# jiaozihao18/LC-Rec

Hardware: AMD Instinct MI355X
Metric: item-embeddings/sec through 4-level RQ encode+assign (higher is better)
Workload: dtype f32; 1 GPU; C3 synthetic 1M x 768-d, 4x256 codes; items_per_gpu=1000000, in_dim=768, e_dim=32, levels=4, codes_per_level=256, chunk_pipelines=1, bytes_per_item=3104

## Files before the change

### lc-rec_amd/csrc/gemm_f32.hip

```cpp
#include "common.h"

#include <stdlib.h>

namespace lcrec {

#ifdef LCREC_GEMM_STAMP
__device__ unsigned long long g_stamps[8][64][4];
__device__ unsigned long long g_marks[8][4];
#define LCREC_MARK(slot)                                                                           \
    do {                                                                                           \
        if (blockIdx.x == 8 && lane == 0) {                                                        \
            unsigned long long t_;                                                                 \
            asm volatile("s_memtime %0\n\ts_waitcnt lgkmcnt(0)" : "=s"(t_)::"memory");           \
            g_marks[wave][slot] = t_;                                                              \
        }                                                                                          \
    } while (0)
#define LCREC_STAMP(slot)                                                                          \
    do {                                                                                           \
        if (blockIdx.x == 8 && lane == 0 && 2 * u + half < 64) {                                   \
            unsigned long long t_;                                                                 \
            asm volatile("s_memtime %0\n\ts_waitcnt lgkmcnt(0)" : "=s"(t_)::"memory");           \
            g_stamps[wave][2 * u + half][slot] = t_;                                               \
        }                                                                                          \
    } while (0)
// ... 759 lines not shown
            for (int r = 0; r < 16; ++r) acc[i][j][r] = 0.f;

    const int nk = K / BKT;
    float *my_a = As0 + grp * GM * LDT;

    const __amdgpu_buffer_rsrc_t a_rsrc = tile_rsrc(A, m0, M, GM, K);
    const __amdgpu_buffer_rsrc_t w_rsrc = tile_rsrc(W, w_row0, N, 64, K);
    const int t_g = ((gt / KG) * K + (gt % KG) * 8) * 4;
    const int pass_g = RPI * K * 4;
    const uint32_t t_s = (uint32_t)(((gt / KG) * LDT + (gt % KG) * 8) * 4);
    uint32_t a_s[ITA], w_s[2][ITW];
#pragma unroll
    for (int it = 0; it < ITA; ++it) a_s[it] = lds_addr(my_a) + t_s + it * RPI * LDT * 4;
#pragma unroll
    for (int b = 0; b < 2; ++b)
#pragma unroll
        for (int it = 0; it < ITW; ++it) w_s[b][it] = lds_addr(Ws0 + b * BN * LDT + grp * 64 * LDT) + t_s + it * RPI * LDT * 4;

    f32x4 ra[ITA][2], rw[ITW][2];
    auto load_a = [&](int kt) {
#pragma unroll
        for (int it = 0; it < ITA; ++it) {
            const int so = kt * (BKT * 4) + it * pass_g;
            ra[it][0] = buffer_load_f32x4(a_rsrc, t_g, so);
            ra[it][1] = buffer_load_f32x4(a_rsrc, t_g + 16, so);
        }
    };
    auto load_w = [&](int kt) {
#pragma unroll
        for (int it = 0; it < ITW; ++it) {
            const int so = kt * (BKT * 4) + it * pass_g;
            rw[it][0] = buffer_load_f32x4(w_rsrc, t_g, so);
            rw[it][1] = buffer_load_f32x4(w_rsrc, t_g + 16, so);
        }
    };
    auto store_a = [&]() {
#pragma unroll
        for (int it = 0; it < ITA; ++it) lds_store_deint8(a_s[it], ra[it][0], ra[it][1]);
    };
    auto store_w = [&](int buf) {
#pragma unroll
        for (int it = 0; it < ITW; ++it) lds_store_deint8(w_s[buf][it], rw[it][0], rw[it][1]);
    };
    auto lds_drain = [&]() { asm volatile("s_waitcnt lgkmcnt(0)" ::: "memory"); };

    load_w(0);
    store_w(0);
    load_a(0);
    if (grp == 0) {
        store_a();
    } else if (nk > 1) {
        load_w(1);
    }
    lds_drain();
    __syncthreads();
    LCREC_MARK(1);

    const float *a_base = my_a + (wm * 64 + (lane & 31)) * LDT + (lane >> 5) * 4;
    const int w_off = (wn * 64 + (lane & 31)) * LDT + (lane >> 5) * 4;

    auto mfma_group = [&](const f32x4 (&af)[2], const f32x4 (&wf)[2]) {
#pragma unroll
        for (int q = 0; q < 4; ++q)
#pragma unroll
            for (int i = 0; i < 2; ++i)
#pragma unroll
                for (int j = 0; j < 2; ++j)
                    acc[i][j] = __builtin_amdgcn_mfma_f32_32x32x2f32(af[i][q], wf[j][q], acc[i][j], 0, 0, 0);
    };

    auto phase = [&](auto par_c, auto half_c, int u) {
        constexpr int PAR = decltype(par_c)::value, half = decltype(half_c)::value;
        if (grp == half) {
            LCREC_STAMP(0);
            const float *w_base = Ws0 + PAR * BN * LDT + w_off;
            f32x4 af[2][2], wf[2][2];
            auto frags = [&](int buf, int g) {
#pragma unroll
                for (int i = 0; i < 2; ++i) {
                    af[buf][i] = *reinterpret_cast<const f32x4 *>(a_base + i * 32 * LDT + g * 8);
                    wf[buf][i] = *reinterpret_cast<const f32x4 *>(w_base + i * 32 * LDT + g * 8);
                }
            };
            auto reads_then_mfmas = [&]() {
                __builtin_amdgcn_sched_group_barrier(0x100, 4, 0);
                __builtin_amdgcn_sched_group_barrier(0x008, 16, 0);
            };
            frags(0, 0);
            frags(1, 1);
            if (half == 0) {
                if (u + 1 < nk) { load_a(u + 1); load_w(u + 1); }
            } else {
                if (u + 1 < nk) load_a(u + 1);
                if (u + 2 < nk) load_w(u + 2);
            }
            __builtin_amdgcn_sched_barrier(0);
            mfma_group(af[0], wf[0]);
            __builtin_amdgcn_sched_barrier(0);
            frags(0, 2);
            mfma_group(af[1], wf[1]);
            reads_then_mfmas();
            __builtin_amdgcn_sched_barrier(0);
            frags(1, 3);
            mfma_group(af[0], wf[0]);
            reads_then_mfmas();
            __builtin_amdgcn_sched_barrier(0);
            LCREC_STAMP(1);
            __syncthreads();
            LCREC_STAMP(2);
            __builtin_amdgcn_s_setprio(3);
            mfma_group(af[1], wf[1]);
            __builtin_amdgcn_s_setprio(0);
            LCREC_STAMP(3);
        } else {
            LCREC_STAMP(0);
            store_a();
            store_w(PAR ^ 1);
            lds_drain();
            LCREC_STAMP(1);
            __syncthreads();
            LCREC_STAMP(2);
        }
    };

    for (int u = 0; u < nk; u += 2) {
        phase(IntC<0>{}, IntC<0>{}, u);
        phase(IntC<0>{}, IntC<1>{}, u);
        if (u + 1 < nk) {
            phase(IntC<1>{}, IntC<0>{}, u + 1);
            phase(IntC<1>{}, IntC<1>{}, u + 1);
        }
    }

    LCREC_MARK(2);
    float *stg = my_a + w4 * 32 * LDK;
#pragma unroll
    for (int j = 0; j < 2; ++j)
#pragma unroll
        for (int i = 0; i < 2; ++i)
            store_tile_32x32(acc[i][j], stg, lane, C, m0 + wm * 64 + i * 32, M, n0 + wn * 64 + j * 32, N, bias, bn_scale,
                             bn_shift, relu);
    LCREC_MARK(3);
}

typedef unsigned u32x4_t __attribute__((ext_vector_type(4)));

template <bool HAS_BN>
__global__ __launch_bounds__(512) void linear_fwd_pp3_kernel(
    const float *__restrict__ A, const float *__restrict__ W, const float *__restrict__ bias,
    const float *__restrict__ bn_scale, const float *__restrict__ bn_shift, float *__restrict__ C,
    int64_t M, int N, int K, int relu, int bn_blocks, int bm_blocks, int total_virtual, int xcd_order)
{
    constexpr int GM = 128, BN = 128, LDT = LDK;
    constexpr int STEADY = 0, HEAD0 = 1, HEAD_S0 = 2, HEAD_S8 = 10, TAIL0 = 11, TAIL1 = 12;
    extern __shared__ __attribute__((aligned(16))) float pp3_lds[];
    float *As0 = pp3_lds;
    float *Ws0 = As0 + 2 * GM * LDT;
    float *Ep0 = Ws0 + 2 * BN * LDT;

    const int tid = threadIdx.x, lane = tid & 63;
    const int wave = __builtin_amdgcn_readfirstlane(tid >> 6);
    const int grp = wave >> 2, w4 = wave & 3, wm = w4 >> 1, wn = w4 & 1;
    const int gt = tid & 255;
    const int nk = K / BK;
    float *my_a = As0 + grp * GM * LDT;
    float *patch = Ep0 + wave * 32 * LDT;

    auto tile_of = [&](int t, int64_t &o_m0, int &o_n0, int &o_arows, int &o_wrows) __attribute__((always_inline)) -> bool {
        int64_t bm;
        int bn;
        if (xcd_order) {
            const int xcd = t & 7, j = t >> 3;
            const int panels = (bm_blocks - xcd + 7) >> 3;
            if (j >= panels * bn_blocks) return false;
            bm = (int64_t)(j / bn_blocks) * 8 + xcd;
            bn = j % bn_blocks;
        } else {
            if (t >= bm_blocks * bn_blocks) return false;
            bm = t / bn_blocks;
            bn = t % bn_blocks;
        }
        o_m0 = bm * (2 * GM) + grp * GM;
        o_n0 = bn * BN;
        const int64_t ar = M - o_m0, wr = (int64_t)N - (o_n0 + grp * 64);
        o_arows = __builtin_amdgcn_readfirstlane((int)(ar < 0 ? 0 : (ar > GM ? GM : ar)));
        o_wrows = __builtin_amdgcn_readfirstlane((int)(wr < 0 ? 0 : (wr > 64 ? 64 : wr)));
        return true;
    };
    auto next_tile = [&](int t, int64_t &o_m0, int &o_n0, int &o_arows, int &o_wrows) __attribute__((always_inline)) -> int {
        for (t += gridDim.x; t < total_virtual; t += gridDim.x)
            if (tile_of(t, o_m0, o_n0, o_arows, o_wrows)) return t;
        return total_virtual;
    };

    int64_t cur_m0 = 0, nxt_m0 = 0, prv_m0 = 0;
    int cur_n0 = 0, nxt_n0 = 0, prv_n0 = 0, cur_ar = 0, nxt_ar = 0, prv_ar = 0, cur_wr = 0, nxt_wr = 0;
    int t = blockIdx.x;
    if (!tile_of(t, cur_m0, cur_n0, cur_ar, cur_wr)) t = next_tile(t, cur_m0, cur_n0, cur_ar, cur_wr);
    if (t >= total_virtual) return;
    int has_next = 0, have_prev = 0;

    const int t_g = ((gt >> 2) * K + (gt & 3) * 8) * 4;
    const int pass_g = 64 * K * 4;
    const uint32_t t_s = (uint32_t)(((gt >> 2) * LDT + (gt & 3) * 8) * 4);
    const uint32_t a_s0 = lds_addr(my_a) + t_s, a_s1 = a_s0 + 64 * LDT * 4;
    const uint32_t w_s[2] = {lds_addr(Ws0 + grp * 64 * LDT) + t_s, lds_addr(Ws0 + BN * LDT + grp * 64 * LDT) + t_s};

    __amdgpu_buffer_rsrc_t cur_a = tile_rsrc(A, cur_m0, M, GM, K), cur_w = tile_rsrc(W, cur_n0 + grp * 64, N, 64, K);
    __amdgpu_buffer_rsrc_t nxt_a = cur_a, nxt_w = cur_w;

    f32x4 ra[2][2], rw[2];
    auto load_a = [&](__amdgpu_buffer_rsrc_t r, int kt) __attribute__((always_inline)) {
        const int so = kt * (BK * 4);
        ra[0][0] = buffer_load_f32x4(r, t_g, so);
        ra[0][1] = buffer_load_f32x4(r, t_g + 16, so);
        ra[1][0] = buffer_load_f32x4(r, t_g, so + pass_g);
        ra[1][1] = buffer_load_f32x4(r, t_g + 16, so + pass_g);
    };
    auto load_w = [&](__amdgpu_buffer_rsrc_t r, int kt) __attribute__((always_inline)) {
        const int so = kt * (BK * 4);
        rw[0] = buffer_load_f32x4(r, t_g, so);
        rw[1] = buffer_load_f32x4(r, t_g + 16, so);
    };
    auto store_a = [&]() __attribute__((always_inline)) {
        lds_store_deint8(a_s0, ra[0][0], ra[0][1]);
        lds_store_deint8(a_s1, ra[1][0], ra[1][1]);
    };
    auto store_w = [&](int buf) __attribute__((always_inline)) { lds_store_deint8(w_s[buf], rw[0], rw[1]); };
    auto lds_drain = [&]() __attribute__((always_inline)) { asm volatile("s_waitcnt lgkmcnt(0)" ::: "memory"); };
    auto lds_barrier = [&]() __attribute__((always_inline)) { asm volatile("s_waitcnt lgkmcnt(0)\n\ts_barrier" ::: "memory"); };

    struct EpiConst { float b[2], sc[2], sh[2]; };
    auto load_epi = [&](EpiConst &e, int n0) __attribute__((always_inline)) {
#pragma unroll
        for (int j = 0; j < 2; ++j) {
            const int col = n0 + wn * 64 + j * 32 + (lane & 31);
            e.b[j] = bias ? bias[col] : 0.f;
            e.sc[j] = HAS_BN ? bn_scale[col] : 1.f;
            e.sh[j] = HAS_BN ? bn_shift[col] : 0.f;
        }
    };
    auto epi_math = [&](f32x16 (&dst)[2][2], const f32x16 (&src)[2][2], const EpiConst &e) __attribute__((always_inline)) {
#pragma unroll
        for (int i = 0; i < 2; ++i)
#pragma unroll
            for (int j = 0; j < 2; ++j)
#pragma unroll
                for (int r = 0; r < 16; ++r) {
                    float v = src[i][j][r] + e.b[j];
                    if (HAS_BN) v = __builtin_fmaf(v, e.sc[j], e.sh[j]);
                    if (relu) v = (v > 0.f) ? v : 0.f;
                    dst[i][j][r] = v;
                }
    };
    uint32_t patch_w = lds_addr(patch) + (uint32_t)((4 * (lane >> 5) * LDT + (lane & 31)) * 4);
    uint32_t patch_r = lds_addr(patch) + (uint32_t)(((lane >> 3) * LDT + (lane & 7) * 4) * 4);
    int c_voff = ((lane >> 3) * N + (lane & 7) * 4) * 4;
    asm volatile("" : "+v"(patch_w), "+v"(patch_r), "+v"(c_voff));
    auto epi_patch = [&](const f32x16 &v, auto hf_c) __attribute__((always_inline)) {
        constexpr int hf = decltype(hf_c)::value;
        const uint32_t pw = patch_w;
#define LCREC_PATCH_W(R)                                                                                         \
        asm volatile("ds_write_b32 %0, %1 offset:%2" ::"v"(pw), "v"(v[8 * hf + (R)]),                            \
                     "n"((((R) & 3) + 8 * ((8 * hf + (R)) >> 2)) * LDT * 4) : "memory")
        LCREC_PATCH_W(0); LCREC_PATCH_W(1); LCREC_PATCH_W(2); LCREC_PATCH_W(3);
        LCREC_PATCH_W(4); LCREC_PATCH_W(5); LCREC_PATCH_W(6); LCREC_PATCH_W(7);
#undef LCREC_PATCH_W
    };
    auto epi_send = [&](auto i_c, auto j_c, auto hf_c, int64_t t_m0, int t_n0, int rows) __attribute__((always_inline)) {
        constexpr int i = decltype(i_c)::value, j = decltype(j_c)::value, hf = decltype(hf_c)::value;
        const int extent = rows > 0 ? ((rows - 1) * N + BN) * 4 : 0;
        const __amdgpu_buffer_rsrc_t c_rsrc =
            __builtin_amdgcn_make_buffer_rsrc(C + t_m0 * (int64_t)N + t_n0, 0, extent, 0x00020000);
        f32x4 q[2];
        asm volatile("s_waitcnt lgkmcnt(0)\n\t"
                     "ds_read_b128 %0, %2 offset:%3\n\t"
                     "ds_read_b128 %1, %2 offset:%4\n\t"
                     "s_waitcnt lgkmcnt(0)"
                     : "=&v"(q[0]), "=&v"(q[1])
                     : "v"(patch_r), "n"((2 * hf) * 8 * LDT * 4), "n"((2 * hf + 1) * 8 * LDT * 4)
                     : "memory");
#pragma unroll
        for (int p = 0; p < 2; ++p) {
            const int soff = ((wm * 64 + i * 32 + 8 * (2 * hf + p)) * N + wn * 64 + j * 32) * 4;
            __builtin_amdgcn_raw_buffer_store_b128(__builtin_bit_cast(u32x4_t, q[p]), c_rsrc, c_voff, soff, 0);
            asm volatile("s_nop 3" ::: "memory");
        }
    };
    auto epi_store = [&](const f32x16 &v, auto i_c, auto j_c, auto hf_c, int64_t t_m0, int t_n0, int rows) __attribute__((always_inline)) {
        epi_patch(v, hf_c);
        epi_send(i_c, j_c, hf_c, t_m0, t_n0, rows);
    };

    load_w(cur_w, 0);
    store_w(0);
    load_a(cur_a, 0);
    if (grp == 0) {
        store_a();
    } else {
        load_w(cur_w, 1);
    }
    lds_drain();
    lds_barrier();

    const float *a_base = my_a + (wm * 64 + (lane & 31)) * LDT + (lane >> 5) * 4;
    const int w_off = (wn * 64 + (lane & 31)) * LDT + (lane >> 5) * 4;

    f32x16 acc[2][2], prev[2][2];
    EpiConst ec;
    auto phase = [&](auto par_c, auto half_c, auto mode_c, int u) __attribute__((always_inline)) {
        constexpr int PAR = decltype(par_c)::value, half = decltype(half_c)::value, MODE = decltype(mode_c)::value;
        if (grp == half) {
            LCREC_STAMP(0);
            const float *w_base = Ws0 + PAR * BN * LDT + w_off;
            f32x4 af[2][2], wf[2][2];
            auto frags = [&](int buf, int g) {
#pragma unroll
                for (int i = 0; i < 2; ++i) {
                    af[buf][i] = *reinterpret_cast<const f32x4 *>(a_base + i * 32 * LDT + g * 8);
                    wf[buf][i] = *reinterpret_cast<const f32x4 *>(w_base + i * 32 * LDT + g * 8);
                }
            };
            auto mfma_group = [&](const f32x4 (&a2)[2], const f32x4 (&w2)[2]) {
#pragma unroll
                for (int q = 0; q < 4; ++q)
#pragma unroll
                    for (int i = 0; i < 2; ++i)
#pragma unroll
                        for (int j = 0; j < 2; ++j)
                            acc[i][j] = __builtin_amdgcn_mfma_f32_32x32x2f32(a2[i][q], w2[j][q], acc[i][j], 0, 0, 0);
            };
            auto reads_then_mfmas = [&]() {
                __builtin_amdgcn_sched_group_barrier(0x100, 4, 0);
                __builtin_amdgcn_sched_group_barrier(0x008, 16, 0);
            };
            if constexpr (MODE == HEAD0) {
                if (have_prev) epi_math(prev, acc, ec);
                load_epi(ec, cur_n0);
#pragma unroll
                for (int i = 0; i < 2; ++i)
#pragma unroll
                    for (int j = 0; j < 2; ++j)
#pragma unroll
                        for (int r = 0; r < 16; ++r) acc[i][j][r] = 0.f;
            }
            frags(0, 0);
            frags(1, 1);
            __builtin_amdgcn_sched_barrier(0);
            if constexpr (MODE == TAIL0) {
                if (half == 0) {
                    load_a(cur_a, u + 1);
                    load_w(cur_w, u + 1);
                } else {
                    load_a(cur_a, u + 1);
                    if (has_next) load_w(nxt_w, 0);
                }
            } else if constexpr (MODE == TAIL1) {
                if (has_next) {
                    load_a(nxt_a, 0);
                    load_w(nxt_w, half == 0 ? 0 : 1);
                }
            } else {
                load_a(cur_a, u + 1);
                load_w(cur_w, half == 0 ? u + 1 : u + 2);
            }
            __builtin_amdgcn_sched_barrier(0);
            mfma_group(af[0], wf[0]);
            __builtin_amdgcn_sched_barrier(0);
            if constexpr (MODE >= HEAD_S0 && MODE < HEAD_S8) {
                if (have_prev) {
                    constexpr int s = (MODE - HEAD_S0) >> 1, hf = (MODE - HEAD_S0) & 1;
                    epi_patch(prev[s >> 1][s & 1], IntC<hf>{});
                }
            }
            __builtin_amdgcn_sched_barrier(0);
            frags(0, 2);
            mfma_group(af[1], wf[1]);
            reads_then_mfmas();
            __builtin_amdgcn_sched_barrier(0);
            frags(1, 3);
            mfma_group(af[0], wf[0]);
            reads_then_mfmas();
            __builtin_amdgcn_sched_barrier(0);
            LCREC_STAMP(1);
            lds_barrier();
            LCREC_STAMP(2);
            __builtin_amdgcn_s_setprio(3);
            mfma_group(af[1], wf[1]);
            __builtin_amdgcn_s_setprio(0);
            LCREC_STAMP(3);
        } else {
            LCREC_STAMP(0);
            store_a();
            store_w(PAR ^ 1);
            lds_drain();
            LCREC_STAMP(1);
            constexpr int PIECE = MODE - HEAD_S0 - (half == 0 ? 1 : 0);
            if constexpr (MODE >= HEAD_S0 && MODE <= HEAD_S8 && PIECE >= 0 && PIECE < 8) {
                if (have_prev) {
                    constexpr int s = PIECE >> 1, hf = PIECE & 1;
                    epi_send(IntC<(s >> 1)>{}, IntC<(s & 1)>{}, IntC<hf>{}, prv_m0, prv_n0, prv_ar);
                }
            }
            LCREC_STAMP(3);
            lds_barrier();
            LCREC_STAMP(2);
        }
    };
    auto pair = [&](auto par_c, auto mode_c, int u) __attribute__((always_inline)) {
        phase(par_c, IntC<0>{}, mode_c, u);
        phase(par_c, IntC<1>{}, mode_c, u);
    };
    auto finish = [&]() __attribute__((always_inline)) {
        epi_math(acc, acc, ec);
        epi_store(acc[0][0], IntC<0>{}, IntC<0>{}, IntC<0>{}, cur_m0, cur_n0, cur_ar);
        epi_store(acc[0][0], IntC<0>{}, IntC<0>{}, IntC<1>{}, cur_m0, cur_n0, cur_ar);
        epi_store(acc[0][1], IntC<0>{}, IntC<1>{}, IntC<0>{}, cur_m0, cur_n0, cur_ar);
        epi_store(acc[0][1], IntC<0>{}, IntC<1>{}, IntC<1>{}, cur_m0, cur_n0, cur_ar);
        epi_store(acc[1][0], IntC<1>{}, IntC<0>{}, IntC<0>{}, cur_m0, cur_n0, cur_ar);
        epi_store(acc[1][0], IntC<1>{}, IntC<0>{}, IntC<1>{}, cur_m0, cur_n0, cur_ar);
        epi_store(acc[1][1], IntC<1>{}, IntC<1>{}, IntC<0>{}, cur_m0, cur_n0, cur_ar);
        epi_store(acc[1][1], IntC<1>{}, IntC<1>{}, IntC<1>{}, cur_m0, cur_n0, cur_ar);
    };

    for (;;) {
        const int tn = next_tile(t, nxt_m0, nxt_n0, nxt_ar, nxt_wr);
        has_next = tn < total_virtual ? 1 : 0;
        pair(IntC<0>{}, IntC<HEAD0>{}, 0);
        pair(IntC<1>{}, IntC<HEAD_S0 + 0>{}, 1);
        pair(IntC<0>{}, IntC<HEAD_S0 + 1>{}, 2);
        pair(IntC<1>{}, IntC<HEAD_S0 + 2>{}, 3);
        pair(IntC<0>{}, IntC<HEAD_S0 + 3>{}, 4);
        pair(IntC<1>{}, IntC<HEAD_S0 + 4>{}, 5);
        pair(IntC<0>{}, IntC<HEAD_S0 + 5>{}, 6);
        pair(IntC<1>{}, IntC<HEAD_S0 + 6>{}, 7);
        pair(IntC<0>{}, IntC<HEAD_S0 + 7>{}, 8);
        pair(IntC<1>{}, IntC<HEAD_S8>{}, 9);
        for (int u = 10; u < nk - 2; u += 2) {
            pair(IntC<0>{}, IntC<STEADY>{}, u);
            pair(IntC<1>{}, IntC<STEADY>{}, u + 1);
        }
        nxt_a = tile_rsrc(A, nxt_m0, M, GM, K);
        nxt_w = tile_rsrc(W, nxt_n0 + grp * 64, N, 64, K);
        pair(IntC<0>{}, IntC<TAIL0>{}, nk - 2);
        pair(IntC<1>{}, IntC<TAIL1>{}, nk - 1);
        if (!has_next) { finish(); break; }
        prv_m0 = cur_m0; prv_n0 = cur_n0; prv_ar = cur_ar;
        cur_m0 = nxt_m0; cur_n0 = nxt_n0; cur_ar = nxt_ar; cur_wr = nxt_wr; cur_a = nxt_a; cur_w = nxt_w;
        t = tn;
        have_prev = 1;
    }
}

constexpr int S16_BM = 32, S16_BN = 64, S16_LDN = 72, S16_RING = 4;

template <bool TB>
__global__ __launch_bounds__(256) void linear_s16_kernel(const float *__restrict__ A, const float *__restrict__ W,
                                                         const float *__restrict__ bias, const float *__restrict__ bn_scale,
                                                         const float *__restrict__ bn_shift, float *__restrict__ C, int64_t M, int N,
                                                         int K, int relu, int bn_blocks)
{
    constexpr int A_FLOATS = S16_BM * LDK, W_FLOATS = TB ? BK * S16_LDN : S16_BN * LDK, BUF = A_FLOATS + W_FLOATS;
    __shared__ __attribute__((aligned(16))) float smem[2 * BUF];
    const int tid = threadIdx.x, lane = tid & 63, wave = tid >> 6;
    const int wm = wave >> 1, wn = wave & 1, r16 = lane & 15, q = lane >> 4;
    const int64_t bm = blockIdx.x / bn_blocks;
    const int bn = blockIdx.x % bn_blocks;
    const int64_t m0 = bm * S16_BM;
    const int n0 = bn * S16_BN;
    const int nk = K / BK;

    const __amdgpu_buffer_rsrc_t a_rsrc = tile_rsrc(A, m0, M, S16_BM, K);
    const __amdgpu_buffer_rsrc_t w_rsrc = TB ? __builtin_amdgcn_make_buffer_rsrc(const_cast<float *>(W), 0, (int)((int64_t)K * N * 4), 0x00020000)
                                             : tile_rsrc(W, n0, N, S16_BN, K);
    struct Regs { f32x4 a, w[2]; };
    struct Frag { f32x4 a[2], b[2][2]; };
    constexpr unsigned SOFF_OUT = 0x7fffff00u;
    const int arow = tid >> 3, akq = tid & 7;
    const int wkk = tid >> 4, wn4 = tid & 15;
    const bool w_in = !TB || n0 + wn4 * 4 < N;
    const int a_vo = (arow * K + akq * 4) * 4;
    const int w_vo0 = TB ? (w_in ? (int)(((int64_t)wkk * N + n0 + wn4 * 4) * 4) : 0x7fffff00) : a_vo;
    const int w_vo1 = TB ? (w_in ? (int)(((int64_t)(wkk + 16) * N + n0 + wn4 * 4) * 4) : 0x7fffff00) : a_vo + 32 * K * 4;
    auto load_piece = [&](Regs &g, int kt, bool live, auto piece_c) {
        constexpr int piece = decltype(piece_c)::value;
        const unsigned so = live ? (TB && piece > 0 ? (unsigned)((int64_t)kt * BK * N * 4) : (unsigned)(kt * (BK * 4))) : SOFF_OUT;
        if constexpr (piece == 0) g.a = buffer_load_f32x4(a_rsrc, a_vo, (int)so);
        else if constexpr (piece == 1) g.w[0] = buffer_load_f32x4(w_rsrc, w_vo0, (int)so);
        else g.w[1] = buffer_load_f32x4(w_rsrc, w_vo1, (int)so);
    };
    const uint32_t a_st = (uint32_t)((arow * LDK + akq) * 4);
    const uint32_t wk_st = (uint32_t)((A_FLOATS + wkk * S16_LDN + wn4 * 4) * 4);
    auto store_piece = [&](const Regs &g, int buf, auto piece_c) {
        constexpr int piece = decltype(piece_c)::value;
        const uint32_t base = lds_addr(smem) + (uint32_t)(buf * BUF * 4);
        if constexpr (piece < 2) {
            const uint32_t ad = base + a_st + piece * 64;
            asm volatile("ds_write2_b32 %0, %1, %2 offset1:8" ::"v"(ad), "v"(g.a[2 * piece]), "v"(g.a[2 * piece + 1]) : "memory");
        } else if constexpr (TB) {
            const uint32_t ad = base + wk_st;
            if constexpr (piece < 4) asm volatile("ds_write_b128 %0, %1" ::"v"(ad + (uint32_t)((piece - 2) * 16 * S16_LDN * 4)), "v"(g.w[piece - 2]) : "memory");
        } else {
            constexpr int j = (piece - 2) >> 1, h = (piece - 2) & 1;
            const uint32_t ad = base + (uint32_t)(A_FLOATS * 4) + a_st + (uint32_t)(j * 32 * LDK * 4) + h * 64;
            asm volatile("ds_write2_b32 %0, %1, %2 offset1:8" ::"v"(ad), "v"(g.w[j][2 * h]), "v"(g.w[j][2 * h + 1]) : "memory");
        }
    };
    const float *a_fr = smem + (16 * wm + r16) * LDK + q * 8;
    const float *w_fr = smem + A_FLOATS + (32 * wn + r16) * LDK + q * 8;
    const float *wk_fr = smem + A_FLOATS + q * S16_LDN + 32 * wn + r16;
    auto frag_read = [&](Frag &f, int buf, auto slot_c) {
        constexpr int slot = decltype(slot_c)::value;
        if constexpr (slot < 2) {
            f.a[slot] = *reinterpret_cast<const f32x4 *>(a_fr + buf * BUF + slot * 4);
        } else {
            constexpr int cb = (slot - 2) >> 1, h = (slot - 2) & 1;
            if constexpr (TB) {
#pragma unroll
                for (int s = 0; s < 4; ++s) f.b[h][cb][s] = wk_fr[buf * BUF + (4 * s + 16 * h) * S16_LDN + 16 * cb];
            } else {
                f.b[h][cb] = *reinterpret_cast<const f32x4 *>(w_fr + buf * BUF + cb * 16 * LDK + h * 4);
            }
        }
    };

    f32x4 acc[2] = {{0.f, 0.f, 0.f, 0.f}, {0.f, 0.f, 0.f, 0.f}};
    Frag fa, fb;
    Regs ring[S16_RING];
    if (nk > 0) {
        static_for<S16_RING>([&](auto j_c) {
            constexpr int j = decltype(j_c)::value;
            static_for<3>([&](auto p_c) { load_piece(ring[j], j, j < nk, p_c); });
        });
        static_for<6>([&](auto p_c) { store_piece(ring[0], 0, p_c); });
        static_for<6>([&](auto p_c) { store_piece(ring[1], 1, p_c); });
        asm volatile("s_waitcnt lgkmcnt(0)" ::: "memory");
        static_for<3>([&](auto p_c) { load_piece(ring[0], S16_RING, S16_RING < nk, p_c); });
        __syncthreads();
        static_for<6>([&](auto s_c) { frag_read(fa, 0, s_c); });
        asm volatile("s_waitcnt lgkmcnt(0)" ::: "memory");
        __syncthreads();
    }
    auto k_tile = [&](int kt, const Frag &fc, Frag &fn, Regs &r_free, const Regs &r_next, auto cur_c) {
        constexpr int cur = decltype(cur_c)::value;
        const bool live = kt + S16_RING + 1 < nk;
        static_for<16>([&](auto s_c) {
            constexpr int s = decltype(s_c)::value, cb = s & 1, ks = s >> 1, h = ks >> 2, sq = ks & 3;
            acc[cb] = __builtin_amdgcn_mfma_f32_16x16x4f32(fc.a[h][sq], fc.b[h][cb][sq], acc[cb], 0, 0, 0);
            __builtin_amdgcn_sched_barrier(0);
            if constexpr (s < 6) frag_read(fn, cur ^ 1, IntC<s>{});
            if constexpr (s >= 6 && s < 9) load_piece(r_free, kt + S16_RING + 1, live, IntC<s - 6>{});
            if constexpr (s >= 9 && s < 15) store_piece(r_next, cur, IntC<s - 9>{});
            __builtin_amdgcn_sched_barrier(0);
        });
        asm volatile("s_waitcnt lgkmcnt(0)" ::: "memory");
        __syncthreads();
    };
    for (int kt = 0; kt < nk; kt += S16_RING) {
        static_for<S16_RING>([&](auto u_c) {
            constexpr int u = decltype(u_c)::value;
            if (u == 0 || kt + u < nk) {
                if constexpr (u % 2 == 0) k_tile(kt + u, fa, fb, ring[(u + 1) % S16_RING], ring[(u + 2) % S16_RING], IntC<0>{});
                else k_tile(kt + u, fb, fa, ring[(u + 1) % S16_RING], ring[(u + 2) % S16_RING], IntC<1>{});
            }
        });
    }

    const bool has_bn = bn_scale != nullptr;
#pragma unroll
    for (int cb = 0; cb < 2; ++cb) {
        const int col = n0 + 32 * wn + 16 * cb + r16;
        if (col >= N) continue;
        const float bj = bias ? bias[col] : 0.f;
        const float sc = has_bn ? bn_scale[col] : 1.f, sh = has_bn ? bn_shift[col] : 0.f;
#pragma unroll
        for (int r = 0; r < 4; ++r) {
            const int64_t row = m0 + 16 * wm + 4 * q + r;
            if (row >= M) continue;
            float t = acc[cb][r] + bj;
            if (has_bn) t = __builtin_fmaf(t, sc, sh);
            if (relu) t = t > 0.f ? t : 0.f;
            C[row * (int64_t)N + col] = t;
        }
    }
}

static int launch_s16(const float *A, const float *W, const float *b, const float *sc, const float *sh, int relu, float *C, int64_t M,
                      int N, int K, bool kmajor_w, hipStream_t stream)
{
    const int64_t bm_blocks = (M + S16_BM - 1) / S16_BM;
    const int bn_blocks = (N + S16_BN - 1) / S16_BN;
    const int64_t grid = bm_blocks * bn_blocks;
    if (grid > 0x7fffffffLL) return fail(LCREC_EINVAL, "linear (32 x 64 tiles): grid too large");
    TraceScope trace(K_LINEAR_32x64, stream);
    if (kmajor_w) hipLaunchKernelGGL(linear_s16_kernel<true>, dim3((unsigned)grid), dim3(256), 0, stream, A, W, b, sc, sh, C, M, N, K, relu, bn_blocks);
    else hipLaunchKernelGGL(linear_s16_kernel<false>, dim3((unsigned)grid), dim3(256), 0, stream, A, W, b, sc, sh, C, M, N, K, relu, bn_blocks);
    return check_launch("linear_s16_kernel");
}

static bool use_s16_tiles(int64_t M, int N, int K)
{
    static const int mode = [] { const char *e = getenv("LCREC_GEMM_S16"); return e ? atoi(e) : -1; }();
    static const int limit = [] { const char *e = getenv("LCREC_GEMM_S16_TILES"); return e ? atoi(e) : 128; }();
    if (mode == 0 || K % BK != 0 || K < BK || N % 4 != 0 || (int64_t)K * 4 * (M + 64) >= (1ll << 31) || (int64_t)K * N * 4 >= (1ll << 31)) return false;
    if (mode == 1) return true;
    return ((M + 63) / 64) * ((N + 63) / 64) <= limit;
}

static int launch_pp2(dim3 grid, hipStream_t stream, const float *x, const float *W, const float *b, const float *sc,
                      const float *sh, float *y, int64_t n, int out_dim, int in_dim, int relu, int bn_blocks, int bm_blocks,
                      int xcd_order)
{
    constexpr size_t lds = (size_t)(2 * 128 + 2 * 128) * (BK + 4) * sizeof(float);
    static const hipError_t attr = hipFuncSetAttribute(reinterpret_cast<const void *>(linear_fwd_pp2_kernel),
                                                       hipFuncAttributeMaxDynamicSharedMemorySize, (int)lds);
    if (attr != hipSuccess) return fail(LCREC_EHIP, "linear_forward: hipFuncSetAttribute(%zu): %s", lds, hipGetErrorString(attr));
    hipLaunchKernelGGL(linear_fwd_pp2_kernel, grid, dim3(512), lds, stream, x, W, b, sc, sh, y, n, out_dim, in_dim, relu,
                       bn_blocks, bm_blocks, xcd_order);
    return LCREC_OK;
}

static int launch_pp3(int total_virtual, hipStream_t stream, const float *x, const float *W, const float *b, const float *sc,
                      const float *sh, float *y, int64_t n, int out_dim, int in_dim, int relu, int bn_blocks, int bm_blocks,
                      int xcd_order)
{
    constexpr size_t lds = (size_t)(2 * 128 + 2 * 128 + 8 * 32) * LDK * sizeof(float);
    static const int cus = [] {
        int dev = 0, v = 0;
        if (hipGetDevice(&dev) != hipSuccess || hipDeviceGetAttribute(&v, hipDeviceAttributeMultiprocessorCount, dev) != hipSuccess) v = 256;
        return v > 8 ? v / 8 * 8 : 8;
    }();
    static const hipError_t attr0 = hipFuncSetAttribute(reinterpret_cast<const void *>(linear_fwd_pp3_kernel<false>),
                                                        hipFuncAttributeMaxDynamicSharedMemorySize, (int)lds);
    static const hipError_t attr1 = hipFuncSetAttribute(reinterpret_cast<const void *>(linear_fwd_pp3_kernel<true>),
                                                        hipFuncAttributeMaxDynamicSharedMemorySize, (int)lds);
    if (attr0 != hipSuccess || attr1 != hipSuccess)
        return fail(LCREC_EHIP, "linear_forward: hipFuncSetAttribute(%zu): %s", lds, hipGetErrorString(attr0 != hipSuccess ? attr0 : attr1));
    const int grid = total_virtual < cus ? total_virtual : cus;
    if (sc)
        hipLaunchKernelGGL(linear_fwd_pp3_kernel<true>, dim3((unsigned)grid), dim3(512), lds, stream, x, W, b, sc, sh, y, n, out_dim,
                           in_dim, relu, bn_blocks, bm_blocks, total_virtual, xcd_order);
    else
        hipLaunchKernelGGL(linear_fwd_pp3_kernel<false>, dim3((unsigned)grid), dim3(512), lds, stream, x, W, b, sc, sh, y, n, out_dim,
                           in_dim, relu, bn_blocks, bm_blocks, total_virtual, xcd_order);
    return LCREC_OK;
}

static int launch_linear_pp(const float *x, int64_t n, int in_dim, const float *W, const float *b, const float *sc,
                            const float *sh, int relu, int out_dim, float *y, int xcd_order, hipStream_t stream)
{
    const int64_t bm_blocks = (n + 255) / 256;
    const int bn_blocks = (out_dim + 127) / 128;
    const int64_t grid = xcd_order ? ((bm_blocks + 7) / 8) * 8 * bn_blocks : bm_blocks * bn_blocks;
    if (grid > 0x7fffffffLL) return fail(LCREC_EINVAL, "linear_forward: grid too large (n=%lld)", (long long)n);
    TraceScope trace(K_LINEAR_PP, stream);
    static const int pp3 = [] { const char *e = getenv("LCREC_GEMM_PP3"); return e ? atoi(e) : 1; }();
    int rc;
    if (pp3 && in_dim % 64 == 0 && in_dim >= 12 * BK && out_dim % 128 == 0 && (int64_t)out_dim * 4 * 128 < (1ll << 31))
        rc = launch_pp3((int)grid, stream, x, W, b, sc, sh, y, n, out_dim, in_dim, relu, bn_blocks, (int)bm_blocks, xcd_order);
    else
        rc = launch_pp2(dim3((unsigned)grid), stream, x, W, b, sc, sh, y, n, out_dim, in_dim, relu, bn_blocks, (int)bm_blocks,
                        xcd_order);
    return rc ? rc : check_launch("linear_fwd_pp2_kernel");
}

template <int WAVES_M, int WAVES_N, int TM, int TN>
static int launch_linear(const float *x, int64_t n, int in_dim, const float *W, const float *b,
                         const float *sc, const float *sh, int relu, int out_dim, float *y,
                         hipStream_t stream)
{
    constexpr int BM = WAVES_M * TM * 32, BN = WAVES_N * TN * 32;
    const int64_t bm_blocks = (n + BM - 1) / BM;
    const int bn_blocks = (out_dim + BN - 1) / BN;
    static const int tune = [] { const char *e = getenv("LCREC_GEMM_TUNE"); return (e ? atoi(e) : 1) & 1; }();
    const int64_t grid = (tune & 1) ? ((bm_blocks + 7) / 8) * 8 * bn_blocks : bm_blocks * bn_blocks;
    if (grid > 0x7fffffffLL) return fail(LCREC_EINVAL, "linear_forward: grid too large (n=%lld)", (long long)n);
    TraceScope trace(BM == 64 ? K_LINEAR_64x64 : BN == 128 ? K_LINEAR_128x128 : BN == 64 ? K_LINEAR_128x64 : K_LINEAR_128x32, stream);
    static const int fast = [] { const char *e = getenv("LCREC_GEMM_FAST"); return e ? atoi(e) : 1; }();
    if (fast && in_dim % BK == 0 && (int64_t)in_dim * 4 * (BM + 64) < (1ll << 31))
        hipLaunchKernelGGL((linear_fwd_kernel<WAVES_M, WAVES_N, TM, TN, true>), dim3((unsigned)grid), dim3(256), 0,
                           stream, x, W, b, sc, sh, y, n, out_dim, in_dim, relu, bn_blocks, (int)bm_blocks, tune, 1 << 30,
                           (int64_t)0);
    else
        hipLaunchKernelGGL((linear_fwd_kernel<WAVES_M, WAVES_N, TM, TN, false>), dim3((unsigned)grid), dim3(256), 0,
                           stream, x, W, b, sc, sh, y, n, out_dim, in_dim, relu, bn_blocks, (int)bm_blocks, tune, 1 << 30,
                           (int64_t)0);
    return check_launch("linear_fwd_kernel");
}

__global__ __launch_bounds__(256) void splitk_reduce_kernel(const float *__restrict__ partial, int splits, int64_t total4,
                                                          float *__restrict__ out)
{
    const int64_t q = (int64_t)blockIdx.x * 256 + threadIdx.x;
    if (q >= total4) return;
    const f32x4 *p = reinterpret_cast<const f32x4 *>(partial);
    f32x4 acc = p[q];
    for (int s = 1; s < splits; ++s) acc = acc + p[(int64_t)s * total4 + q];
    reinterpret_cast<f32x4 *>(out)[q] = acc;
}

static bool wide_tiles_fill(int64_t M, int N) { return ((M + 63) / 64) * ((N + 127) / 128) >= 256; }

template <int WAVES_M, int WAVES_N, int TM, int TN, bool TA>
static int launch_kmajor(const float *A, const float *B, int64_t M, int N, int K, float *C, int splits, float *partial,
                         hipStream_t stream)
{
    constexpr int BM = WAVES_M * TM * 32, BN = WAVES_N * TN * 32;
    const int64_t bm_blocks = (M + BM - 1) / BM;
    const int bn_blocks = (N + BN - 1) / BN;
    const int64_t grid = ((bm_blocks + 7) / 8) * 8 * bn_blocks;
    if (grid > 0x7fffffffLL) return fail(LCREC_EINVAL, "linear_backward: grid too large");
    const int nk = (K + BK - 1) / BK;
    const int per = splits > 1 ? (nk + splits - 1) / splits : 1 << 30;
    TraceScope trace(BM == 64 ? K_LINEAR_64x64 : BN == 128 ? K_LINEAR_128x128 : BN == 64 ? K_LINEAR_128x64 : K_LINEAR_128x32, stream);
    hipLaunchKernelGGL((linear_fwd_kernel<WAVES_M, WAVES_N, TM, TN, true, TA, true>), dim3((unsigned)grid, (unsigned)(splits > 1 ? splits : 1)),
                       dim3(256), 0, stream, A, B, (const float *)nullptr, (const float *)nullptr, (const float *)nullptr,
                       splits > 1 ? partial : C, M, N, K, 0, bn_blocks, (int)bm_blocks, 1, per, splits > 1 ? M * (int64_t)N : (int64_t)0);
    if (splits > 1) {
        const int64_t total4 = M * (int64_t)N / 4;
        hipLaunchKernelGGL(splitk_reduce_kernel, dim3((unsigned)((total4 + 255) / 256)), dim3(256), 0, stream, partial, splits, total4, C);
    }
    return check_launch("linear_fwd_kernel (k-major operands)");
}

static int kmajor_shape(int64_t M, int N)
{
    if (N > 64) return ((M + 127) / 128) * ((N + 127) / 128) >= 512 ? 1 : (wide_tiles_fill(M, N) ? 4 : 0);
    return N > 32 ? ((M + 127) / 128 < 256 ? 0 : 2) : 3;
}

template <bool TA>
static int gemm_kmajor(const float *A, const float *B, int64_t M, int N, int K, float *C, int splits, float *partial,
                       hipStream_t stream)
{
    if constexpr (!TA) {
        if (splits <= 1 && use_s16_tiles(M, N, K))
            return launch_s16(A, B, nullptr, nullptr, nullptr, 0, C, M, N, K, true, stream);
    }
    switch (kmajor_shape(M, N)) {
    case 0: return launch_kmajor<2, 2, 1, 1, TA>(A, B, M, N, K, C, splits, partial, stream);
    case 1: return launch_kmajor<2, 2, 2, 2, TA>(A, B, M, N, K, C, splits, partial, stream);
    case 2: return launch_kmajor<4, 1, 1, 2, TA>(A, B, M, N, K, C, splits, partial, stream);
    case 4: return launch_kmajor<2, 2, 1, 2, TA>(A, B, M, N, K, C, splits, partial, stream);
    default: return launch_kmajor<4, 1, 1, 1, TA>(A, B, M, N, K, C, splits, partial, stream);
    }
}

int linear_backward_splits(int64_t n, int in_dim, int out_dim)
{
    static const int cap = [] { const char *e = getenv("LCREC_GEMM_SPLITK"); return e ? atoi(e) : 16; }();
    const int shape = kmajor_shape(out_dim, in_dim);
    const int bm = shape == 0 ? 64 : 128, bn = shape == 0 ? 64 : shape == 1 ? 128 : shape == 2 ? 64 : 32;
    const int64_t tiles = ((out_dim + bm - 1) / bm) * (int64_t)((in_dim + bn - 1) / bn);
    const int64_t nk = (n + BK - 1) / BK;
    int64_t s = 512 / (tiles > 0 ? tiles : 1);
    if (s > nk / 4) s = nk / 4;
    if (s > cap) s = cap;
    if (s < 2) return 1;
    const int64_t per = (nk + s - 1) / s;
    return (int)((nk + per - 1) / per);
}

size_t linear_backward_workspace(int64_t n, int in_dim, int out_dim)
{
    const int s = linear_backward_splits(n, in_dim, out_dim);
    return s > 1 ? (size_t)s * out_dim * in_dim * sizeof(float) : 0;
}

int linear_backward(const float *gy, const float *x, const float *W, int64_t n, int in_dim, int out_dim, float *gx, float *gw,
                    void *workspace, size_t workspace_bytes, hipStream_t stream)
{
    if (n == 0) return LCREC_OK;
    if (!gy || (gx && !W) || (gw && !x)) return fail(LCREC_EINVAL, "linear_backward: NULL pointer");
    if (n < 0 || in_dim <= 0 || out_dim <= 0) return fail(LCREC_EINVAL, "linear_backward: bad shape");
    if (in_dim % 4 != 0 || out_dim % 4 != 0)
        return fail(LCREC_EUNSUPPORTED, "linear_backward: in_dim=%d / out_dim=%d must be multiples of 4", in_dim, out_dim);
    if (((uintptr_t)gy | (uintptr_t)x | (uintptr_t)W) & 15) return fail(LCREC_EINVAL, "linear_backward: operands must be 16-byte aligned");
    const int64_t widest = in_dim > out_dim ? in_dim : out_dim;
    if ((n + 64) * widest * 4 >= (1ll << 31) || (int64_t)out_dim * in_dim * 4 >= (1ll << 31))
// ... 239 lines not shown
```

Baseline: 16.65 million items/s.

## Swap MFMA operands to store GEMM epilogue directly, dropping LDS transpose patch

Swaps the A/W operands of the 32x32x2 f32 MFMA so each lane's accumulator holds four consecutive output columns. The epilogue can then write 128-bit stores straight from registers instead of staging through a per-wave LDS patch buffer. Bias and BN constants are now loaded as vectors through buffer loads; for the BN variant they are loaded inside the epilogue math. This removes the ds_write/ds_read transpose traffic and shrinks LDS per block. The cost is strided row stores per lane and extra global loads for the BN constants.

```diff
diff --git a/lc-rec_amd/csrc/gemm_f32.hip b/lc-rec_amd/csrc/gemm_f32.hip
--- a/lc-rec_amd/csrc/gemm_f32.hip
+++ b/lc-rec_amd/csrc/gemm_f32.hip
@@ -935,11 +935,10 @@
     int64_t M, int N, int K, int relu, int bn_blocks, int bm_blocks, int total_virtual, int xcd_order)
 {
     constexpr int GM = 128, BN = 128, LDT = LDK;
-    constexpr int STEADY = 0, HEAD0 = 1, HEAD_S0 = 2, HEAD_S8 = 10, TAIL0 = 11, TAIL1 = 12;
+    constexpr int STEADY = 0, HEAD0 = 1, HEAD_S0 = 2, HEAD_SN = 10, TAIL0 = 11, TAIL1 = 12;
     extern __shared__ __attribute__((aligned(16))) float pp3_lds[];
     float *As0 = pp3_lds;
     float *Ws0 = As0 + 2 * GM * LDT;
-    float *Ep0 = Ws0 + 2 * BN * LDT;
 
     const int tid = threadIdx.x, lane = tid & 63;
     const int wave = __builtin_amdgcn_readfirstlane(tid >> 6);
@@ -947,7 +946,6 @@
     const int gt = tid & 255;
     const int nk = K / BK;
     float *my_a = As0 + grp * GM * LDT;
-    float *patch = Ep0 + wave * 32 * LDT;
 
     auto tile_of = [&](int t, int64_t &o_m0, int &o_n0, int &o_arows, int &o_wrows) __attribute__((always_inline)) -> bool {
         int64_t bm;
@@ -1013,66 +1011,63 @@
     auto lds_drain = [&]() __attribute__((always_inline)) { asm volatile("s_waitcnt lgkmcnt(0)" ::: "memory"); };
     auto lds_barrier = [&]() __attribute__((always_inline)) { asm volatile("s_waitcnt lgkmcnt(0)\n\ts_barrier" ::: "memory"); };
 
-    struct EpiConst { float b[2], sc[2], sh[2]; };
+    struct EpiConst { f32x4 b[HAS_BN ? 1 : 2][4]; };
+    auto col_rsrc = [&](const float *p) __attribute__((always_inline)) {
+        return __builtin_amdgcn_make_buffer_rsrc(const_cast<float *>(p), 0, p ? N * 4 : 0, 0x00020000);
+    };
+    int col_voff = (wn * 64 + 4 * (lane >> 5)) * 4;
+    asm volatile("" : "+v"(col_voff));
     auto load_epi = [&](EpiConst &e, int n0) __attribute__((always_inline)) {
 #pragma unroll
+        for (int j = 0; j < 2; ++j)
+#pragma unroll
+            for (int g = 0; g < 4; ++g)
+                if (!HAS_BN) e.b[j][g] = buffer_load_f32x4(col_rsrc(bias), col_voff, (n0 + 32 * j + 8 * g) * 4);
+    };
+    auto epi_math = [&](f32x16 (&dst)[2][2], const f32x16 (&src)[2][2], const EpiConst &e, int n0) __attribute__((always_inline)) {
+        int vo = col_voff;
+#pragma unroll
         for (int j = 0; j < 2; ++j) {
-            const int col = n0 + wn * 64 + j * 32 + (lane & 31);
-            e.b[j] = bias ? bias[col] : 0.f;
-            e.sc[j] = HAS_BN ? bn_scale[col] : 1.f;
-            e.sh[j] = HAS_BN ? bn_shift[col] : 0.f;
-        }
-    };
-    auto epi_math = [&](f32x16 (&dst)[2][2], const f32x16 (&src)[2][2], const EpiConst &e) __attribute__((always_inline)) {
-#pragma unroll
-        for (int i = 0; i < 2; ++i)
-#pragma unroll
-            for (int j = 0; j < 2; ++j)
-#pragma unroll
-                for (int r = 0; r < 16; ++r) {
-                    float v = src[i][j][r] + e.b[j];
-                    if (HAS_BN) v = __builtin_fmaf(v, e.sc[j], e.sh[j]);
-                    if (relu) v = (v > 0.f) ? v : 0.f;
-                    dst[i][j][r] = v;
+            if (HAS_BN && j == 1) asm volatile("" : "+v"(vo) : "v"(dst[0][0]), "v"(dst[1][0]));
+#pragma unroll
+            for (int g = 0; g < 4; ++g) {
+                f32x4 b = e.b[HAS_BN ? 0 : j][g], sc = {1.f, 1.f, 1.f, 1.f}, sh = {0.f, 0.f, 0.f, 0.f};
+                if (HAS_BN) {
+                    const int so = (n0 + 32 * j + 8 * g) * 4;
+                    b = buffer_load_f32x4(col_rsrc(bias), vo, so);
+                    sc = buffer_load_f32x4(col_rsrc(bn_scale), vo, so);
+                    sh = buffer_load_f32x4(col_rsrc(bn_shift), vo, so);
                 }
-    };
-    uint32_t patch_w = lds_addr(patch) + (uint32_t)((4 * (lane >> 5) * LDT + (lane & 31)) * 4);
-    uint32_t patch_r = lds_addr(patch) + (uint32_t)(((lane >> 3) * LDT + (lane & 7) * 4) * 4);
-    int c_voff = ((lane >> 3) * N + (lane & 7) * 4) * 4;
-    asm volatile("" : "+v"(patch_w), "+v"(patch_r), "+v"(c_voff));
-    auto epi_patch = [&](const f32x16 &v, auto hf_c) __attribute__((always_inline)) {
-        constexpr int hf = decltype(hf_c)::value;
-        const uint32_t pw = patch_w;
-#define LCREC_PATCH_W(R)                                                                                         \
-        asm volatile("ds_write_b32 %0, %1 offset:%2" ::"v"(pw), "v"(v[8 * hf + (R)]),                            \
-                     "n"((((R) & 3) + 8 * ((8 * hf + (R)) >> 2)) * LDT * 4) : "memory")
-        LCREC_PATCH_W(0); LCREC_PATCH_W(1); LCREC_PATCH_W(2); LCREC_PATCH_W(3);
-        LCREC_PATCH_W(4); LCREC_PATCH_W(5); LCREC_PATCH_W(6); LCREC_PATCH_W(7);
-#undef LCREC_PATCH_W
-    };
-    auto epi_send = [&](auto i_c, auto j_c, auto hf_c, int64_t t_m0, int t_n0, int rows) __attribute__((always_inline)) {
-        constexpr int i = decltype(i_c)::value, j = decltype(j_c)::value, hf = decltype(hf_c)::value;
+#pragma unroll
+                for (int i = 0; i < 2; ++i)
+#pragma unroll
+                    for (int r = 0; r < 4; ++r) {
+                        float v = src[i][j][4 * g + r] + b[r];
+                        if (HAS_BN) v = __builtin_fmaf(v, sc[r], sh[r]);
+                        if (relu) v = (v > 0.f) ? v : 0.f;
+                        dst[i][j][4 * g + r] = v;
+                    }
+            }
+        }
+    };
+    int c_voff = ((lane & 31) * N + (lane >> 5) * 4) * 4;
+    asm volatile("" : "+v"(c_voff));
+    auto out_rsrc = [&](int64_t t_m0, int t_n0, int rows) __attribute__((always_inline)) {
         const int extent = rows > 0 ? ((rows - 1) * N + BN) * 4 : 0;
-        const __amdgpu_buffer_rsrc_t c_rsrc =
-            __builtin_amdgcn_make_buffer_rsrc(C + t_m0 * (int64_t)N + t_n0, 0, extent, 0x00020000);
-        f32x4 q[2];
-        asm volatile("s_waitcnt lgkmcnt(0)\n\t"
-                     "ds_read_b128 %0, %2 offset:%3\n\t"
-                     "ds_read_b128 %1, %2 offset:%4\n\t"
-                     "s_waitcnt lgkmcnt(0)"
-                     : "=&v"(q[0]), "=&v"(q[1])
-                     : "v"(patch_r), "n"((2 * hf) * 8 * LDT * 4), "n"((2 * hf + 1) * 8 * LDT * 4)
-                     : "memory");
-#pragma unroll
-        for (int p = 0; p < 2; ++p) {
-            const int soff = ((wm * 64 + i * 32 + 8 * (2 * hf + p)) * N + wn * 64 + j * 32) * 4;
-            __builtin_amdgcn_raw_buffer_store_b128(__builtin_bit_cast(u32x4_t, q[p]), c_rsrc, c_voff, soff, 0);
-            asm volatile("s_nop 3" ::: "memory");
-        }
-    };
-    auto epi_store = [&](const f32x16 &v, auto i_c, auto j_c, auto hf_c, int64_t t_m0, int t_n0, int rows) __attribute__((always_inline)) {
-        epi_patch(v, hf_c);
-        epi_send(i_c, j_c, hf_c, t_m0, t_n0, rows);
+        return __builtin_amdgcn_make_buffer_rsrc(C + t_m0 * (int64_t)N + t_n0, 0, extent, 0x00020000);
+    };
+    auto epi_send = [&](const f32x16 &v, __amdgpu_buffer_rsrc_t c_rsrc, auto i_c, auto j_c, auto g_c) __attribute__((always_inline)) {
+        constexpr int i = decltype(i_c)::value, j = decltype(j_c)::value, g = decltype(g_c)::value;
+        const int soff = ((wm * 64 + i * 32) * N + wn * 64) * 4;
+        const f32x4 q = __builtin_shufflevector(v, v, 4 * g, 4 * g + 1, 4 * g + 2, 4 * g + 3);
+        __builtin_amdgcn_raw_buffer_store_b128(__builtin_bit_cast(u32x4_t, q), c_rsrc, c_voff + (j * 32 + 8 * g) * 4, soff, 0);
+        asm volatile("s_nop 3" ::: "memory");
+    };
+    auto epi_piece = [&](const f32x16 (&src)[2][2], auto piece_c, int64_t t_m0, int t_n0, int rows) __attribute__((always_inline)) {
+        constexpr int piece = decltype(piece_c)::value, s = piece >> 1, hf = piece & 1;
+        const __amdgpu_buffer_rsrc_t c_rsrc = out_rsrc(t_m0, t_n0, rows);
+        epi_send(src[s >> 1][s & 1], c_rsrc, IntC<(s >> 1)>{}, IntC<(s & 1)>{}, IntC<2 * hf>{});
+        epi_send(src[s >> 1][s & 1], c_rsrc, IntC<(s >> 1)>{}, IntC<(s & 1)>{}, IntC<2 * hf + 1>{});
     };
 
     load_w(cur_w, 0);
@@ -1111,14 +1106,14 @@
                     for (int i = 0; i < 2; ++i)
 #pragma unroll
                         for (int j = 0; j < 2; ++j)
-                            acc[i][j] = __builtin_amdgcn_mfma_f32_32x32x2f32(a2[i][q], w2[j][q], acc[i][j], 0, 0, 0);
+                            acc[i][j] = __builtin_amdgcn_mfma_f32_32x32x2f32(w2[j][q], a2[i][q], acc[i][j], 0, 0, 0);
             };
             auto reads_then_mfmas = [&]() {
                 __builtin_amdgcn_sched_group_barrier(0x100, 4, 0);
                 __builtin_amdgcn_sched_group_barrier(0x008, 16, 0);
             };
             if constexpr (MODE == HEAD0) {
-                if (have_prev) epi_math(prev, acc, ec);
+                if (have_prev) epi_math(prev, acc, ec, prv_n0);
                 load_epi(ec, cur_n0);
 #pragma unroll
                 for (int i = 0; i < 2; ++i)
@@ -1150,13 +1145,6 @@
             __builtin_amdgcn_sched_barrier(0);
             mfma_group(af[0], wf[0]);
             __builtin_amdgcn_sched_barrier(0);
-            if constexpr (MODE >= HEAD_S0 && MODE < HEAD_S8) {
-                if (have_prev) {
-                    constexpr int s = (MODE - HEAD_S0) >> 1, hf = (MODE - HEAD_S0) & 1;
-                    epi_patch(prev[s >> 1][s & 1], IntC<hf>{});
-                }
-            }
-            __builtin_amdgcn_sched_barrier(0);
             frags(0, 2);
             mfma_group(af[1], wf[1]);
             reads_then_mfmas();
@@ -1178,12 +1166,8 @@
             store_w(PAR ^ 1);
             lds_drain();
             LCREC_STAMP(1);
-            constexpr int PIECE = MODE - HEAD_S0 - (half == 0 ? 1 : 0);
-            if constexpr (MODE >= HEAD_S0 && MODE <= HEAD_S8 && PIECE >= 0 && PIECE < 8) {
-                if (have_prev) {
-                    constexpr int s = PIECE >> 1, hf = PIECE & 1;
-                    epi_send(IntC<(s >> 1)>{}, IntC<(s & 1)>{}, IntC<hf>{}, prv_m0, prv_n0, prv_ar);
-                }
+            if constexpr (MODE >= HEAD_S0 && MODE < HEAD_SN) {
+                if (have_prev) epi_piece(prev, IntC<MODE - HEAD_S0>{}, prv_m0, prv_n0, prv_ar);
             }
             LCREC_STAMP(3);
             lds_barrier();
@@ -1195,15 +1179,8 @@
         phase(par_c, IntC<1>{}, mode_c, u);
     };
     auto finish = [&]() __attribute__((always_inline)) {
-        epi_math(acc, acc, ec);
-        epi_store(acc[0][0], IntC<0>{}, IntC<0>{}, IntC<0>{}, cur_m0, cur_n0, cur_ar);
-        epi_store(acc[0][0], IntC<0>{}, IntC<0>{}, IntC<1>{}, cur_m0, cur_n0, cur_ar);
-        epi_store(acc[0][1], IntC<0>{}, IntC<1>{}, IntC<0>{}, cur_m0, cur_n0, cur_ar);
-        epi_store(acc[0][1], IntC<0>{}, IntC<1>{}, IntC<1>{}, cur_m0, cur_n0, cur_ar);
-        epi_store(acc[1][0], IntC<1>{}, IntC<0>{}, IntC<0>{}, cur_m0, cur_n0, cur_ar);
-        epi_store(acc[1][0], IntC<1>{}, IntC<0>{}, IntC<1>{}, cur_m0, cur_n0, cur_ar);
-        epi_store(acc[1][1], IntC<1>{}, IntC<1>{}, IntC<0>{}, cur_m0, cur_n0, cur_ar);
-        epi_store(acc[1][1], IntC<1>{}, IntC<1>{}, IntC<1>{}, cur_m0, cur_n0, cur_ar);
+        epi_math(acc, acc, ec, cur_n0);
+        static_for<8>([&](auto p_c) { epi_piece(acc, p_c, cur_m0, cur_n0, cur_ar); });
     };
 
     for (;;) {
@@ -1218,7 +1195,7 @@
         pair(IntC<0>{}, IntC<HEAD_S0 + 5>{}, 6);
         pair(IntC<1>{}, IntC<HEAD_S0 + 6>{}, 7);
         pair(IntC<0>{}, IntC<HEAD_S0 + 7>{}, 8);
-        pair(IntC<1>{}, IntC<HEAD_S8>{}, 9);
+        pair(IntC<1>{}, IntC<STEADY>{}, 9);
         for (int u = 10; u < nk - 2; u += 2) {
             pair(IntC<0>{}, IntC<STEADY>{}, u);
             pair(IntC<1>{}, IntC<STEADY>{}, u + 1);
@@ -1407,7 +1384,7 @@
                       const float *sh, float *y, int64_t n, int out_dim, int in_dim, int relu, int bn_blocks, int bm_blocks,
                       int xcd_order)
 {
-    constexpr size_t lds = (size_t)(2 * 128 + 2 * 128 + 8 * 32) * LDK * sizeof(float);
+    constexpr size_t lds = (size_t)(2 * 128 + 2 * 128) * LDK * sizeof(float);
     static const int cus = [] {
         int dev = 0, v = 0;
         if (hipGetDevice(&dev) != hipSuccess || hipDeviceGetAttribute(&v, hipDeviceAttributeMultiprocessorCount, dev) != hipSuccess) v = 256;
```

New measurement: 16.74 million items/s, median of 6. About the same (+0.5%).
